# xu-ji/IIC

Hardware: AMD Instinct MI355X
Metric: paired-images/sec, STL10 96x96 ClusterNet5g+IID_loss (higher is better)
Workload: dtype bf16; 1 GPU; STL10 96x96 ClusterNet5g IID+ (cluster_sobel.py train step), batch 660 pairs/GPU, 5 sub-heads, k=70, bf16 MFMA convs / fp32 stem+heads+loss, fused HIP Adam; global_batch_pairs=660, input=96x96x1 grey -> sobel 2ch, parallelism=dp1, streams=2, launch=hip-graph replay: 6 linear graph segments, the two views on two streams

## Files before the change

iic_amd/csrc/conv_igemm_bd.hip:

```cpp
#include "common.h"
#include "conv_plan.h"
#include "conv_tile.h"
#include "../../include/iic_hip.h"

__device__ __forceinline__ void bd_bload(u32x4& d, const unsigned char* p) {
  asm volatile("global_load_dwordx4 %0, %1, off" : "=v"(d) : "v"(p) : "memory");
}
template <int N>
__device__ __forceinline__ void bd_bwait(u32x4& d) {
  asm volatile("s_waitcnt vmcnt(%1)" : "+v"(d) : "i"(N) : "memory");
}


#define BD_BM 256
#define BD_BN 128
#define BD_THREADS 256
#define BD_PROF_SLOTS 16
#ifndef BD_STORE_UB
#define BD_STORE_UB 8
#endif

template <bool GATHER, int ABL, int MS, int RED, int WN = 2, bool PAD = false>
__device__ __forceinline__ void bd_tile(
    const iic_conv_geom& g, const bf16_t* __restrict__ in, const unsigned char* __restrict__ wfrag,
    bf16_t* __restrict__ out, float* __restrict__ stats, const bf16_t* __restrict__ res_grad,
    const bf16_t* __restrict__ res_act, int accumulate, int lds_a_bytes,
    const bf16_t* __restrict__ red_y, const float* __restrict__ red_coef,
    const bf16_t* __restrict__ red_y2, float* __restrict__ red_stats, float* __restrict__ red_stats2,
    unsigned long long* __restrict__ prof, int blk_in_class, int nwg_class, const bd_blk& B) {
  constexpr int BNT = WN * 64, NWM = 4 / WN;
  constexpr bool CANBLK = !GATHER && MS * 32 * (4 / WN) == 256;
  const bool blk = CANBLK && !PAD && B.bw > 0;
  constexpr int CLD = BNT + 8;
  constexpr bool PROF = (ABL & 128) != 0;
  static_assert(!(PAD && GATHER), "the padded patch is a multi-tap form");
  constexpr bool SWZ = !PAD;
  unsigned long long t_stamp[8];
  unsigned long long t_bsum = 0, t_b0 = 0;
  int t_nb = 0;
  if (PROF) t_stamp[0] = __builtin_readcyclecounter();
  constexpr int BM = MS * 32 * NWM, WR = MS * 32;
  extern __shared__ __attribute__((aligned(16))) unsigned char smem_raw[];
  unsigned char* sA = smem_raw;
  int* s_pin = reinterpret_cast<int*>(smem_raw + lds_a_bytes);
  int* s_pout = s_pin + BM;
  float* s_red = reinterpret_cast<float*>(s_pout + BM);
  unsigned char* s_key = reinterpret_cast<unsigned char*>(s_red + NWM * 2 * BNT);
  bf16_t* sC = reinterpret_cast<bf16_t*>(smem_raw);

  const int tid = threadIdx.x, lane = tid & 63;
  const int wave = __builtin_amdgcn_readfirstlane(tid >> 6);
  const int wm = WN == 2 ? wave >> 1 : wave, wn = WN == 2 ? wave & 1 : 0;
  const int l31 = lane & 31, g5 = lane >> 5;

  const int nt = g.Cout / BNT;
  const int tix = xcd_tile_index(blk_in_class, nwg_class);
  const int mtile = tix / nt, ntile = tix - mtile * nt;
  const int n0 = ntile * BNT;
  const int m0 = mtile * BM;
  const int in_pixels = g.N * g.in_Hp * g.in_Wp;

  int v_tapoff = g.tap_off[lane & (IIC_MAX_TAPS - 1)];
  const int v_tapw = g.tap_w[lane & (IIC_MAX_TAPS - 1)];
  int blk_glo = 0;
  bool blk_full = true;
  if (blk) {
    const int tpi = B.nbx * B.nby;
    const int bn = mtile / tpi, brem = mtile - bn * tpi;
    const int by = brem / B.nbx, bx = brem - by * B.nbx;
    const int y0 = by * B.bh, x0 = bx * B.bw;
    blk_glo = (bn * g.in_Hp + y0 + g.oy) * g.in_Wp + x0 + g.ox;
    blk_full = y0 + B.bh <= g.MY && x0 + B.bw <= g.MX && B.bw * B.bh == BM;
    v_tapoff = (v_tapoff / g.in_Wp) * B.PW + v_tapoff % g.in_Wp;
    if (tid < BM) {
      int ky = tid / B.bw;
      const int kx = tid - ky * B.bw;
      const int y = y0 + ky, x = x0 + kx;
      const bool valid = ky < B.bh && y < g.MY && x < g.MX;
      ky = ky < B.bh ? ky : B.bh - 1;
      s_pin[tid] = ky * B.PW + kx;
      s_pout[tid] = valid ? (bn * g.out_Hp + y + g.py) * g.out_Wp + x + g.px : -1;
    }
  } else if (tid < BM) {
    int pin, pout;
    igemm_row_pixels(g, m0 + tid, pin, pout);
    s_pin[tid] = pin;
    s_pout[tid] = pout;
  }
  __syncthreads();
  const int p_lo = blk ? 0 : s_pin[0];
  const int npix = GATHER ? BM : (blk ? B.npix : (BM >= 192 ? g.NP256 : g.NP));
  const int keyw = blk ? B.PW : g.in_Wp;
  const int jskip = blk ? B.PW - B.bw
                        : ((!GATHER && g.sx == 1 && ((g.in_Wp - g.MX) & 1) == 0) ? g.in_Wp - g.MX : 0);
  auto dense_of = [&](int p) { return p - jskip * (p / keyw); };
  int arow[MS];
  int drow[MS];
#pragma unroll
  for (int ms = 0; ms < MS; ++ms) {
    const int row = wm * WR + ms * 32 + l31;
    const int pr = GATHER ? row : (s_pin[row] - p_lo);
    arow[ms] = SWZ ? pr : pr * ROWB + g5 * 16;
    drow[ms] = (SWZ && !GATHER) ? dense_of(s_pin[row]) : pr;
  }
  if (SWZ && !GATHER && jskip != 0) {
    for (int r = tid; r < npix; r += BD_THREADS) s_key[r] = (unsigned char)((dense_of(p_lo + r) >> 1) & 7);
    __syncthreads();
  }
  const int v_tapd = v_tapoff - jskip * (v_tapoff / keyw);
  const int nblk = (npix * 128 + 1023) >> 10;
  const int dma_rl = lane / 9, dma_pc = min(lane - dma_rl * 9, 7) * 8;
  auto dma_patch = [&](int c0) {
    if (PAD) {
      const int nj = (npix + PT144_ROWS - 1) / PT144_ROWS;
      for (int j = wave; j < nj; j += BD_THREADS / 64) {
        long p = (long)p_lo + j * PT144_ROWS + dma_rl;
        p = p < in_pixels ? p : in_pixels - 1;
        __builtin_amdgcn_global_load_lds(
            (const __attribute__((address_space(1))) void*)(in + (p * g.Cin + c0 + dma_pc)),
            (__attribute__((address_space(3))) void*)(sA + j * PT144_PIECE), 16, 0, 0);
      }
      asm volatile("s_waitcnt vmcnt(0)" ::: "memory");
      return;
    }
    for (int kb = wave; kb < nblk; kb += BD_THREADS / 64) {
      const int q = kb * 64 + lane;
      const int r = q >> 3;
      const int ls = (q & 7) ^ (GATHER ? ((r >> 1) & 7)
                                       : (jskip != 0 ? (int)s_key[r < npix ? r : npix - 1]
                                                     : (((p_lo + r) >> 1) & 7)));
      long p = GATHER ? (long)s_pin[r < BM ? r : BM - 1] : (long)p_lo + r;
      if (blk) {
        const int rc = r < npix ? r : npix - 1;
        const int py = (rc * B.mul) >> 16;
        p = (long)blk_glo + py * g.in_Wp + (rc - py * B.PW);
      }
      p = p < in_pixels ? p : in_pixels - 1;
      __builtin_amdgcn_global_load_lds(
          (const __attribute__((address_space(1))) void*)(in + (p * g.Cin + c0 + ls * 8)),
          (__attribute__((address_space(3))) void*)(sA + kb * 1024), 16, 0, 0);
    }
    asm volatile("s_waitcnt vmcnt(0)" ::: "memory");
  };
  auto a_base = [&](int R, int D) { return R * 128 + (((g5 ^ (D >> 1)) & 1) << 4); };
  auto a_kk = [&](int D) { return ((D >> 2) & 3) << 5; };

  f32x16 acc[MS][2];
#pragma unroll
  for (int ms = 0; ms < MS; ++ms)
#pragma unroll
    for (int ns = 0; ns < 2; ++ns)
#pragma unroll
      for (int r = 0; r < 16; ++r) acc[ms][ns][r] = 0.f;

  const int nchunks = g.Cin >> 6;
  const int ntaps = g.ntaps;
  const int NIT = nchunks * ntaps;
  const long frag_it = (long)(g.Cout >> 5) * 4096;
  const unsigned char* wb0 = wfrag + (long)((n0 + wn * 64) >> 5) * 4096 + lane * 16;
  auto frag_ptr = [&](int tap, int chunk) {
    const int tw = __builtin_amdgcn_readlane(v_tapw, tap);
    return wb0 + ((long)tw * nchunks + chunk) * frag_it;
  };

  if (PROF) t_stamp[1] = __builtin_readcyclecounter();
  u32x4 Bc[4][2];
  {
    const unsigned char* p = frag_ptr(0, 0);
#pragma unroll
    for (int ks = 0; ks < 4; ++ks)
#pragma unroll
      for (int ns = 0; ns < 2; ++ns)
        bd_bload(Bc[ks][ns], p + ns * 4096 + ks * 1024);
  }
  dma_patch(0);
  __syncthreads();
  if (PROF) t_stamp[2] = __builtin_readcyclecounter();

  int tap = 0, chunk = 0;
  bf16x8 a[2][MS];
  int pcur[MS], kcur[MS];
#pragma unroll
  for (int ms = 0; ms < MS; ++ms) {
    const int t0 = GATHER ? 0 : __builtin_amdgcn_readlane(v_tapoff, 0);
    if (SWZ) {
      const int R = arow[ms] + t0;
      const int D = drow[ms] + (GATHER ? 0 : __builtin_amdgcn_readlane(v_tapd, 0));
      pcur[ms] = a_base(R, D);
      kcur[ms] = a_kk(D);
      a[0][ms] = *reinterpret_cast<const bf16x8*>(sA + pcur[ms] + kcur[ms]);
    } else {
      pcur[ms] = arow[ms] + t0 * ROWB;
      kcur[ms] = 0;
      a[0][ms] = *reinterpret_cast<const bf16x8*>(sA + pcur[ms]);
    }
  }
  for (int it = 0; it < NIT; ++it) {
    int tn = tap + 1, cn = chunk;
    if (tn == ntaps) { tn = 0; ++cn; }
    const bool more = (it + 1 < NIT);
    if (!more) { tn = tap; cn = chunk; }
    const unsigned char* nb = (ABL & 2) ? frag_ptr(0, 0) : frag_ptr(tn, cn);
    const int toffn = GATHER ? 0 : __builtin_amdgcn_readlane(v_tapoff, tn);
    const int tdn = GATHER ? 0 : __builtin_amdgcn_readlane(v_tapd, tn);
    int pnext[MS], knext[MS];
#pragma unroll
    for (int ms = 0; ms < MS; ++ms) {
      if (SWZ) {
        const int R = arow[ms] + toffn;
        const int D = drow[ms] + tdn;
        pnext[ms] = a_base(R, D);
        knext[ms] = a_kk(D);
      } else {
        pnext[ms] = arow[ms] + toffn * ROWB;
        knext[ms] = 0;
      }
    }
    auto a_read = [&](int ks, int nxt, int cur, int ms) {
      if (!(ABL & 16)) {
        if (SWZ)
          a[nxt][ms] = (ks < 3) ? *reinterpret_cast<const bf16x8*>(sA + pcur[ms] + (((ks + 1) << 5) ^ kcur[ms]))
                                : *reinterpret_cast<const bf16x8*>(sA + pnext[ms] + knext[ms]);
        else
          a[nxt][ms] = (ks < 3) ? *reinterpret_cast<const bf16x8*>(sA + pcur[ms] + (ks + 1) * 32)
                                : *reinterpret_cast<const bf16x8*>(sA + pnext[ms]);
      } else {
        a[nxt][ms] = a[cur][ms];
      }
    };
#pragma unroll
    for (int ks = 0; ks < 4; ++ks) {
      const int cur = ks & 1, nxt = cur ^ 1;
      bd_bwait<7>(Bc[ks][0]);
      __builtin_amdgcn_sched_barrier(0);
      const bf16x8 b0 = __builtin_bit_cast(bf16x8, Bc[ks][0]);
#pragma unroll
      for (int ms = 0; ms < MS; ++ms) {
        acc[ms][0] = __builtin_amdgcn_mfma_f32_32x32x16_bf16(a[cur][ms], b0, acc[ms][0], 0, 0, 0);
        a_read(ks, nxt, cur, ms);
        __builtin_amdgcn_sched_barrier(0);
      }
      bd_bwait<6>(Bc[ks][1]);
      bd_bload(Bc[ks][0], nb + ks * 1024);
      __builtin_amdgcn_sched_barrier(0);
      const bf16x8 b1 = __builtin_bit_cast(bf16x8, Bc[ks][1]);
#pragma unroll
      for (int ms = 0; ms < MS; ++ms)
        acc[ms][1] = __builtin_amdgcn_mfma_f32_32x32x16_bf16(a[cur][ms], b1, acc[ms][1], 0, 0, 0);
      __builtin_amdgcn_sched_barrier(0);
      bd_bload(Bc[ks][1], nb + 4096 + ks * 1024);
      __builtin_amdgcn_sched_barrier(0);
    }
#pragma unroll
    for (int ms = 0; ms < MS; ++ms) {
      pcur[ms] = pnext[ms];
      kcur[ms] = knext[ms];
    }
    if (more && tn == 0 && !(ABL & 8)) {
      if (PROF) t_b0 = __builtin_readcyclecounter();
      __syncthreads();
      if (!(ABL & 1)) dma_patch(cn * 64);
      __syncthreads();
      if (PROF) { t_bsum += __builtin_readcyclecounter() - t_b0; ++t_nb; }
#pragma unroll
      for (int ms = 0; ms < MS; ++ms)
        a[0][ms] = *reinterpret_cast<const bf16x8*>(sA + pcur[ms] + (SWZ ? kcur[ms] : 0));
    }
    tap = tn;
    chunk = cn;
  }

  asm volatile("s_waitcnt vmcnt(0)" ::: "memory");
  if (PROF) t_stamp[3] = __builtin_readcyclecounter();
  if (ABL & 4) {
    float t = 0.f;
#pragma unroll
    for (int ms = 0; ms < MS; ++ms)
#pragma unroll
      for (int ns = 0; ns < 2; ++ns)
#pragma unroll
        for (int r = 0; r < 16; ++r) t += acc[ms][ns][r];
    if (t == 123.f) out[0] = 1;
    return;
  }
  const bool tail = blk ? !blk_full : igemm_tile_has_invalid(g, m0, BM);
  if (stats && !(ABL & 64)) {
    if (tail) {
#pragma unroll
      for (int ms = 0; ms < MS; ++ms)
#pragma unroll
        for (int r = 0; r < 16; ++r)
          if (s_pout[wm * WR + ms * 32 + mfma32_row(r, lane)] < 0) {
            acc[ms][0][r] = 0.f;
            acc[ms][1][r] = 0.f;
          }
    }
#pragma unroll
    for (int ns = 0; ns < 2; ++ns) {
      f32x2 s2 = {0.f, 0.f}, ss2 = {0.f, 0.f};
#pragma unroll
      for (int ms = 0; ms < MS; ++ms)
#pragma unroll
        for (int r = 0; r < 16; r += 2) {
          const f32x2 v = {acc[ms][ns][r], acc[ms][ns][r + 1]};
          s2 += v;
          ss2 += v * v;
        }
      float s = s2[0] + s2[1], ss = ss2[0] + ss2[1];
      s += __shfl_xor(s, 32, 64);
      ss += __shfl_xor(ss, 32, 64);
      if (lane < 32) {
        const int col = wn * 64 + ns * 32 + lane;
        s_red[(wm * 2 + 0) * BNT + col] = s;
        s_red[(wm * 2 + 1) * BNT + col] = ss;
      }
    }
  }
  __syncthreads();
  if (stats && tid < BNT && !(ABL & 64)) {
    const int stripe = blockIdx.x % IIC_STAT_STRIPES;
    float a0 = 0.f, a1 = 0.f;
#pragma unroll
    for (int q = 0; q < NWM; ++q) {
      a0 += s_red[(q * 2 + 0) * BNT + tid];
      a1 += s_red[(q * 2 + 1) * BNT + tid];
    }
    iic_stat_add(stats, stripe, g.Cout, n0 + tid, 0, a0);
    iic_stat_add(stats, stripe, g.Cout, n0 + tid, 1, a1);
  }
#pragma unroll
  for (int ms = 0; ms < MS; ++ms)
#pragma unroll
    for (int ns = 0; ns < 2; ++ns)
#pragma unroll
      for (int r = 0; r < 16; ++r) {
        const int row = wm * WR + ms * 32 + mfma32_row(r, lane);
        const int col = wn * 64 + ns * 32 + l31;
        sC[row * CLD + col] = f32_to_bf16(acc[ms][ns][r]);
      }
  __syncthreads();
  if (PROF) t_stamp[4] = __builtin_readcyclecounter();
  TileRed tr;
  if (RED) tile_red_zero(tr);
  if (!(ABL & 32))
    igemm_store_tile<BNT, BM, BD_THREADS, 8, RED, (BM == 256 ? BD_STORE_UB : 4)>(sC, s_pout, out, res_grad, res_act, accumulate,
                                                                 g.Cout, n0, tid, red_y, red_coef, red_y2, &tr);
  if (RED)
    igemm_red_finish<BNT, BD_THREADS, RED>(tr, reinterpret_cast<float*>(smem_raw), red_stats, red_stats2,
                                             g.Cout, n0, tid);
  if (PROF && prof && tid == 0) {
    unsigned long long* q = prof + (long)blockIdx.x * BD_PROF_SLOTS;
    const unsigned long long t_end = __builtin_readcyclecounter();
    q[0] = t_stamp[0]; q[1] = t_stamp[1]; q[2] = t_stamp[2]; q[3] = t_stamp[3]; q[4] = t_stamp[4];
    q[5] = t_end; q[6] = t_bsum; q[7] = (unsigned long long)t_nb;
    q[8] = iic_hw_stamp();
    q[9] = (unsigned long long)tix;
    q[10] = __builtin_amdgcn_s_memrealtime();
  }
}

template <bool GATHER, int ABL, int MS, int RED, int WN = 2, bool PAD = false>
__global__ __launch_bounds__(BD_THREADS, ((MS == 4 || WN == 1) ? 2 : 3)) void conv_igemm_bd_kernel(
    const iic_conv_geom g, const bf16_t* __restrict__ in, const unsigned char* __restrict__ wfrag,
    bf16_t* __restrict__ out, float* __restrict__ stats, const bf16_t* __restrict__ res_grad,
    const bf16_t* __restrict__ res_act, int accumulate, int num_mtiles, int lds_a_bytes,
    const bf16_t* __restrict__ red_y, const float* __restrict__ red_coef,
    const bf16_t* __restrict__ red_y2, float* __restrict__ red_stats, float* __restrict__ red_stats2,
    unsigned long long* __restrict__ prof, const bd_blk B) {
  bd_tile<GATHER, ABL, MS, RED, WN, PAD>(g, in, wfrag, out, stats, res_grad, res_act, accumulate, lds_a_bytes, red_y,
                                    red_coef, red_y2, red_stats, red_stats2, prof, (int)blockIdx.x,
                                    num_mtiles * (g.Cout / (WN * 64)), B);
}

__global__ void weight_prep_frag_kernel(const float* __restrict__ w, bf16_t* __restrict__ o, int Co,
                                        int Ci, int T, int mode) {
  const int Nn = mode ? Ci : Co, Kk = mode ? Co : Ci;
  const int n32 = Nn >> 5, nchunks = Kk >> 6;
  const long total = (long)T * Co * Ci;
  for (long i = (long)blockIdx.x * blockDim.x + threadIdx.x; i < total;
       i += (long)gridDim.x * blockDim.x) {
    const int e = (int)(i & 7), lane = (int)((i >> 3) & 63), ks = (int)((i >> 9) & 3);
    long r = i >> 11;
    const int j = (int)(r % n32);
    r /= n32;
    const int kc = (int)(r % nchunks), t = (int)(r / nchunks);
    const int n = j * 32 + (lane & 31), k = kc * 64 + ks * 16 + (lane >> 5) * 8 + e;
    const int co = mode ? k : n, ci = mode ? n : k;
    o[i] = f32_to_bf16(w[((long)co * Ci + ci) * T + t]);
  }
}

IIC_SWITCH(g_p64_enabled, 1, iic_debug_enable_p64)
IIC_SWITCH(g_p64_red, 0, iic_debug_p64_red)

extern "C" {

#ifdef IIC_DEBUG_HOOKS
static unsigned long long* g_bd_prof = nullptr;
IIC_HOOK void iic_debug_bd_prof(void* buf) { g_bd_prof = (unsigned long long*)buf; }
IIC_HOOK int iic_debug_bd_prof_slots(void) { return BD_PROF_SLOTS; }
#else
static constexpr unsigned long long* g_bd_prof = nullptr;
#endif

static long bd_lds(long npix, int rows, int couts, bool pad, bool keys, int* lds_a = nullptr) {
  const long a = pad ? pt144_bytes(npix) : (npix * 128 + 1023) & ~1023L;
  const long c = (long)rows * (couts + 8) * 2;
  const long la = ((a > c ? a : c) + 15) & ~15L;
  if (lds_a) *lds_a = (int)la;
  return la + 2L * rows * 4 + 4L * BD_BN * 4 + (keys ? (npix + 15) & ~15L : 0);
}
static long bd_lds_rows(const iic_conv_geom* g, int ms, int wn = 2, bool pad = false, int* lds_a = nullptr) {
  const int rows = ms * 32 * (4 / wn);
  const long npix = g->ntaps == 1 ? rows : (rows >= 192 ? g->NP256 : g->NP);
  const bool skip = g->ntaps > 1 && g->sx == 1 && ((g->in_Wp - g->MX) & 1) == 0 && g->in_Wp != g->MX;
  return bd_lds(npix, rows, wn * 64, pad, !pad && skip, lds_a);
}
IIC_SWITCH(g_bd_pitch144, IIC_BD_PITCH144, iic_debug_bd_pitch144)
#ifdef IIC_DEBUG_HOOKS
IIC_HOOK int iic_debug_get_bd_pitch144(void) { return g_bd_pitch144; }
#endif
static bool bd_pad_ok(const iic_conv_geom* g, int ms) {
  if (!g_bd_pitch144 || g->ntaps < 2 || g->sx != 1 || g->sy != 1) return false;
  return bd_lds_rows(g, ms, 2, true) <= (ms == 4 ? IIC_LDS_WG2 : IIC_LDS_WG3);
}
IIC_SWITCH(g_bd_w1, 1, iic_debug_bd_w1)
static bool bd_w1_ok(const iic_conv_geom* g) {
  return g_bd_w1 && g->Cout % 64 == 0 && g->Cout % BD_BN != 0 && g->ntaps > 1 && g->NP256 > 0 &&
         bd_lds_rows(g, 2, 1) <= IIC_LDS_BYTES;
}
IIC_SWITCH(g_bd_ms, 0, iic_debug_bd_ms)
static int bd_pick_ms(const iic_conv_geom* g) {
  const bool ok4 = (g->ntaps == 1 || g->NP256 > 0) && bd_lds_rows(g, 4) <= IIC_LDS_BYTES;
  const bool ok2 = (g->ntaps == 1 || g->NP > 0) && bd_lds_rows(g, 2) <= IIC_LDS_BYTES;
  if (g_bd_ms == 4) return ok4 ? 4 : (ok2 ? 2 : 0);
  if (g_bd_ms == 2) return ok2 ? 2 : (ok4 ? 4 : 0);
  if (ok4 && ok2 && g->ntaps > 1) {
    const long M = igemm_rows_host(g);
    if (((M + 255) / 256) * (g->Cout / BD_BN) * 2 <= 512) return 2;
  }
  return ok4 ? 4 : (ok2 ? 2 : 0);
}

IIC_SWITCH(g_bd_blk, 1, iic_debug_bd_blk)
static int bd_block_config(const iic_conv_geom* g, bd_blk* B, int wn) {
  B->bw = 0;
  if (!g_bd_blk || g->ntaps < 2 || g->Cout % (wn * 64) != 0 || g->Cin % 64 != 0) return 0;
  if (g->sy != 1 || g->sx != 1 || g->ty != 1 || g->tx != 1 || g->MY < 32 || g->MX < 32 || g->NP256 <= 0) return 0;
  int mix = 0, miy = 0;
  for (int t = 0; t < g->ntaps; ++t) {
    const int iy = g->tap_off[t] / g->in_Wp, ix = g->tap_off[t] % g->in_Wp;
    if (ix > 8 || iy > 8) return 0;
    mix = ix > mix ? ix : mix;
    miy = iy > miy ? iy : miy;
  }
  if (mix & 1) return 0;
  double best = -1.0;
  int best_bw = 0;
  long best_tiles = 0;
  for (int bw = 8; bw <= 64 && bw <= g->MX; ++bw) {
    const int bh = BD_BM / bw;
    if (bh < 2 || bh > g->MY) continue;
    const long tiles = (long)((g->MX + bw - 1) / bw) * ((g->MY + bh - 1) / bh);
    const long npix = (long)(bw + mix) * (bh + miy);
    if (bd_lds(npix, BD_BM, wn * 64, false, true) > IIC_LDS_WG2 || npix >= 65536 / (bw + mix)) continue;
    const double cost = (double)tiles * (1.0 + 0.5 * (double)npix * 128.0 / 32768.0);
    if (best < 0 || cost < best) { best = cost; best_bw = bw; best_tiles = tiles; }
  }
  if (best < 0) return 0;
  const int bw = best_bw, bh = BD_BM / bw;
  if ((double)g->MY * g->MX < 0.88 * (double)BD_BM * (double)best_tiles) return 0;
  const int npix = (bw + mix) * (bh + miy);
  if (g_bd_blk != 2 && !(bd_lds_rows(g, wn == 2 ? 4 : 2, wn) > IIC_LDS_WG2 || npix * 10 < g->NP256 * 7)) return 0;
  B->bw = bw; B->bh = bh;
  B->nbx = (g->MX + bw - 1) / bw; B->nby = (g->MY + bh - 1) / bh;
  B->PW = bw + mix; B->npix = npix; B->mul = (65536 + B->PW - 1) / B->PW;
  return 1;
}

static bool conv_make_plan(const iic_conv_geom* g, conv_plan* p) {
  *p = conv_plan{};
  if (!g) return false;
  if (g_p64_enabled && iic_p64_plan(g, p)) {
    p->red_ok = g_p64_red != 0;
    return true;
  }
  if (g->Cin % 64 != 0 || g->Cout % 64 != 0 || g->ntaps < 1 || g->ntaps > IIC_MAX_TAPS) return false;
  const int abl = iic_debug_get_ablate();
  if (abl == 0 && g_bd_ms == 0 && iic_pw_plan(g, p)) {
    p->red_ok = true;
    return true;
  }
  p->wn = g->Cout % BD_BN != 0 ? 1 : 2;
  const bool blocked = (p->wn == 1 || abl == 0) && bd_block_config(g, &p->blk, p->wn) != 0;
  if (p->wn == 1) p->ms = (blocked || bd_w1_ok(g)) ? 2 : 0;
  else p->ms = blocked ? 4 : bd_pick_ms(g);
  if (p->ms == 0) {
    *p = conv_plan{};
    return false;
  }
  const int rows = p->ms * 32 * (4 / p->wn);
  p->gather = g->ntaps == 1;
  p->red_ok = !p->gather;
  p->pad = p->wn == 2 && !blocked && abl == 0 && bd_pad_ok(g, p->ms);
  p->mtiles = blocked ? g->N * p->blk.nbx * p->blk.nby : (int)((igemm_rows_host(g) + rows - 1) / rows);
  p->grid = p->mtiles * (g->Cout / (p->wn * 64));
  p->lds = blocked ? bd_lds(p->blk.npix, BD_BM, p->wn * 64, false, true, &p->lds_a)
                   : bd_lds_rows(g, p->ms, p->wn, p->pad, &p->lds_a);
  p->kernel = CONV_BD;
  return true;
}

int iic_conv_igemm_frag_supported(const iic_conv_geom* g) {
  conv_plan p;
  return conv_make_plan(g, &p) ? 1 : 0;
}

int iic_conv_igemm_red_supported(const iic_conv_geom* g) {
  conv_plan p;
  return conv_make_plan(g, &p) && p.red_ok ? 1 : 0;
}

int iic_conv_igemm_frag_red(const iic_conv_geom* g, const void* in, const void* wfrag, void* out,
                            float* stats, const void* res_grad, const void* res_act, int accumulate,
                            const void* red_y, const float* red_coef, const void* red_y2,
                            float* red_stats, float* red_stats2, void* stream);

int iic_conv_igemm_frag(const iic_conv_geom* g, const void* in, const void* wfrag, void* out,
                        float* stats, const void* res_grad, const void* res_act, int accumulate,
                        void* stream) {
  return iic_conv_igemm_frag_red(g, in, wfrag, out, stats, res_grad, res_act, accumulate, nullptr, nullptr,
                                 nullptr, nullptr, nullptr, stream);
}

int iic_conv_igemm_frag_red(const iic_conv_geom* g, const void* in, const void* wfrag, void* out,
                            float* stats, const void* res_grad, const void* res_act, int accumulate,
                            const void* red_y, const float* red_coef, const void* red_y2,
                            float* red_stats, float* red_stats2, void* stream) {
  if (!g || !in || !wfrag || !out) return IIC_ERR_ARG;
  if ((red_y == nullptr) != (red_stats == nullptr) || (red_y2 == nullptr) != (red_stats2 == nullptr) ||
      (red_y2 && !red_y) || (red_coef && !red_y))
    return IIC_ERR_ARG;
  const int red = red_y ? (red_y2 ? 2 : 1) : 0;
  if (!(accumulate & IIC_ACC_PREMASK) && (res_grad == nullptr) != (res_act == nullptr)) return IIC_ERR_ARG;
  conv_plan p;
  if (!conv_make_plan(g, &p)) return IIC_ERR_UNSUPPORTED;
  if (p.kernel == CONV_P64) {
    if (red && !p.red_ok) return IIC_ERR_UNSUPPORTED;
    return iic_p64_launch(g, p, in, wfrag, out, stats, res_grad, res_act, accumulate, red_y, red_coef, red_y2,
                          red_stats, red_stats2, stream);
  }
  if (p.kernel == CONV_PW)
    return iic_pw_launch(g, p, in, wfrag, out, stats, res_grad, res_act, accumulate, red_y, red_coef, red_y2, red_stats,
// ... 136 lines not shown
```

iic_amd/csrc/conv_igemm_p64.hip:

```cpp
#include "common.h"
#include "conv_plan.h"
#include "conv_tile.h"
#include "../../include/iic_hip.h"

#define P64_BM 256
#define P64_BN 64
#define P64_THREADS 512
#define P64_NT 9
#define P64_CLD P64_BN
#define P64_SC_BYTES(BM_) ((BM_) * P64_CLD * 2)
#define P64_NTAB 4
#define P64_TAB_BYTES(BM_) (P64_NTAB * (BM_) * (4 + 2))

struct P64Walk {
  int n, y, x;
};
__device__ __forceinline__ void p64_walk_init(P64Walk& w, const iic_conv_geom& g, int m) {
  const int plane = g.MY * g.MX;
  w.n = m / plane;
  const int r = m - w.n * plane;
  w.y = r / g.MX;
  w.x = r - w.y * g.MX;
}
__device__ __forceinline__ void p64_walk_advance(P64Walk& w, const iic_conv_geom& g, int d_y, int d_x) {
  w.x += d_x;
  w.y += d_y;
  if (w.x >= g.MX) { w.x -= g.MX; ++w.y; }
  while (w.y >= g.MY) { w.y -= g.MY; ++w.n; }
}
__device__ __forceinline__ void p64_walk_pixels(const P64Walk& w, const iic_conv_geom& g, int& pin,
                                                int& pout) {
  const bool valid = w.n < g.N;
  const int n = valid ? w.n : g.N - 1, y = valid ? w.y : g.MY - 1, x = valid ? w.x : g.MX - 1;
  pin = (n * g.in_Hp + y * g.sy + g.oy) * g.in_Wp + x * g.sx + g.ox;
  pout = valid ? (n * g.out_Hp + y * g.ty + g.py) * g.out_Wp + x * g.tx + g.px : -1;
}

template <int ABL, int RED>
__global__ __launch_bounds__(512) void conv_igemm_p64_kernel(
    const iic_conv_geom g, const bf16_t* __restrict__ in, const unsigned char* __restrict__ wfrag,
    bf16_t* __restrict__ out, float* __restrict__ stats, const bf16_t* __restrict__ res_grad,
    const bf16_t* __restrict__ res_act, int accumulate, int num_tiles, int pb_bytes, int max_tap_off,
    const bf16_t* __restrict__ red_y, const float* __restrict__ red_coef,
    const bf16_t* __restrict__ red_y2, float* __restrict__ red_stats, float* __restrict__ red_stats2,
    unsigned long long* __restrict__ prof) {
  constexpr bool PROF = (ABL & 8) != 0;
  constexpr int NW = 8, BM = P64_BM;
  constexpr int NWM = BM / 64;
  constexpr int SC_BYTES = BM * P64_CLD * 2, TAB_ROWS = P64_NTAB * BM;
  unsigned long long ph[6] = {0, 0, 0, 0, 0, 0}, t_a = 0, t_b = 0, t_loop = 0;
  extern __shared__ __attribute__((aligned(16))) unsigned char smem_raw[];
  unsigned char* const sP0 = smem_raw;
  unsigned char* const sP1 = smem_raw + pb_bytes;
  bf16_t* const sC = reinterpret_cast<bf16_t*>(smem_raw + 2 * pb_bytes);
  int* const s_pout = reinterpret_cast<int*>(smem_raw + 2 * pb_bytes + SC_BYTES);
  unsigned short* const s_prow = reinterpret_cast<unsigned short*>(s_pout + TAB_ROWS);
  float* const s_red = reinterpret_cast<float*>(sC);

  constexpr int NTH = NW * 64;
  constexpr int NCO = 1;
  const int tid = threadIdx.x, lane = tid & 63;
  const int wave = __builtin_amdgcn_readfirstlane(tid >> 6);
  const int wm = wave >> 1, wn = wave & 1;
  const int l31 = lane & 31, g5 = lane >> 5;
  const int M = g.N * g.MY * g.MX;
  const int in_pixels = g.N * g.in_Hp * g.in_Wp;

  const int G = gridDim.x;
  const int wl = xcd_tile_index(blockIdx.x, G);
  const int t0 = (int)(((long)wl * num_tiles) / G), t1 = (int)(((long)(wl + 1) * num_tiles) / G);
  if (t0 >= t1) return;

  const int v_tapoff = g.tap_off[lane & (IIC_MAX_TAPS - 1)];
  const int d_y = BM / g.MX, d_x = BM - d_y * g.MX;

  P64Walk wr, w0, w255;
  p64_walk_init(wr, g, t0 * BM + (tid & (BM - 1)));
  p64_walk_init(w0, g, t0 * BM);
  p64_walk_init(w255, g, t0 * BM + BM - 1);
  int plo_q[3], nblk_q[3];
  auto tabulate = [&](int t) {
    int pin, pout, p0, p255, dummy;
    p64_walk_pixels(w0, g, p0, dummy);
    p64_walk_pixels(w255, g, p255, dummy);
    p0 = __builtin_amdgcn_readfirstlane(p0);
    p255 = __builtin_amdgcn_readfirstlane(p255);
    if (tid < BM) {
      p64_walk_pixels(wr, g, pin, pout);
      s_pout[(t & (P64_NTAB - 1)) * BM + tid] = pout;
      s_prow[(t & (P64_NTAB - 1)) * BM + tid] = (unsigned short)(pin - p0);
    }
    p64_walk_advance(wr, g, d_y, d_x);
    p64_walk_advance(w0, g, d_y, d_x);
    p64_walk_advance(w255, g, d_y, d_x);
    plo_q[0] = plo_q[1];
    nblk_q[0] = nblk_q[1];
    plo_q[1] = plo_q[2];
    nblk_q[1] = nblk_q[2];
    plo_q[2] = p0;
    nblk_q[2] = ((p255 + max_tap_off - p0 + 1) * 128 + 1023) >> 10;
  };
  auto dma_issue = [&](unsigned char* dst, int plo, int nblk) {
    for (int blk = wave; blk < nblk; blk += NW) {
      const int q = blk * 64 + lane;
      const int r = q >> 3;
      const int ls = (q & 7) ^ ((r >> 1) & 7);
      int p = plo + r;
      p = p < in_pixels ? p : in_pixels - 1;
      __builtin_amdgcn_global_load_lds(
          (const __attribute__((address_space(1))) void*)(in + ((long)p * 64 + ls * 8)),
          (__attribute__((address_space(3))) void*)(dst + blk * 1024), 16, 0, 0);
    }
  };

  tabulate(t0);
  tabulate(t0 + 1);
  dma_issue(sP0, plo_q[1], nblk_q[1]);
  u32x4 Bw[P64_NT][NCO][4];
#pragma unroll
  for (int tap = 0; tap < P64_NT; ++tap)
#pragma unroll
    for (int c = 0; c < NCO; ++c) {
      const unsigned char* p = wfrag + ((long)g.tap_w[tap] * 2 + wn + c) * 4096 + lane * 16;
#pragma unroll
      for (int ks = 0; ks < 4; ++ks) Bw[tap][c][ks] = *reinterpret_cast<const u32x4*>(p + ks * 1024);
    }
  f32x2 st_s[NCO], st_ss[NCO];
#pragma unroll
  for (int c = 0; c < NCO; ++c) {
    st_s[c] = f32x2{0.f, 0.f};
    st_ss[c] = f32x2{0.f, 0.f};
  }
  TileRed tr;
  if (RED) tile_red_zero(tr);

  if (PROF) t_loop = __builtin_readcyclecounter();
  for (int t = t0; t < t1; ++t) {
    const int par = (t - t0) & 1;
    unsigned char* const sP = par ? sP1 : sP0;
    if (PROF) t_a = __builtin_readcyclecounter();
    asm volatile("s_waitcnt vmcnt(0)" ::: "memory");
    __syncthreads();
    if (PROF) { t_b = __builtin_readcyclecounter(); ph[0] += t_b - t_a; t_a = t_b; }
    const bool spread = RED == 0 && !res_grad && !res_act && !accumulate;
    if (t > t0 && !(ABL & 2) && !spread)
      igemm_store_tile<P64_BN, BM, NTH, 0, RED, (RED ? 1 : 4)>(sC, s_pout + ((t - 1) & (P64_NTAB - 1)) * BM,
                                                            out, res_grad, res_act, accumulate, P64_BN, 0, tid,
                                                            red_y, red_coef, red_y2, &tr);
    if (PROF) { t_b = __builtin_readcyclecounter(); ph[1] += t_b - t_a; t_a = t_b; }
    if (t + 1 < t1 && !(ABL & 1)) dma_issue(par ? sP0 : sP1, plo_q[2], nblk_q[2]);
    tabulate(t + 2);
    if (PROF) { t_b = __builtin_readcyclecounter(); ph[2] += t_b - t_a; t_a = t_b; }
    int R0[2];
#pragma unroll
    for (int ms = 0; ms < 2; ++ms)
      R0[ms] = s_prow[(t & (P64_NTAB - 1)) * BM + wm * 64 + ms * 32 + l31];
    f32x16 acc[2][NCO];
    constexpr int NTAPS = (ABL & 4) ? 1 : P64_NT;
    auto load_a = [&](int tap, bf16x8 (&a)[2][4]) {
      const int toff = __builtin_amdgcn_readlane(v_tapoff, tap);
#pragma unroll
      for (int ms = 0; ms < 2; ++ms) {
        const int R = R0[ms] + toff;
        const int key = (R >> 1) & 7;
        const int base = R * 128 + (((g5 ^ key) & 1) << 4);
        const int kk = (key >> 1) << 5;
#pragma unroll
        for (int ks = 0; ks < 4; ++ks)
          a[ms][ks] = *reinterpret_cast<const bf16x8*>(sP + base + ((ks << 5) ^ kk));
      }
    };
#pragma unroll
    for (int tap = 0; tap < NTAPS; ++tap) {
      bf16x8 a[2][4];
      load_a(tap, a);
      if (spread && t > t0 && !(ABL & 2)) {
        constexpr int SIT = BM * 8 / NTH;
        constexpr int PER = (SIT + P64_NT - 2) / (P64_NT - 1);
#pragma unroll
        for (int q = 0; q < PER; ++q) {
          const int it = (tap - 1) * PER + q;
          if (tap >= 1 && it < SIT) {
            const int idx = tid + it * NTH;
            const int row = idx >> 3, ch = idx & 7;
            const int po = s_pout[((t - 1) & (P64_NTAB - 1)) * BM + row];
            if (po >= 0)
              *reinterpret_cast<uint4*>(out + (long)po * P64_BN + ch * 8) =
                  *reinterpret_cast<const uint4*>(sC + row * P64_CLD + ch * 8);
          }
        }
      }
#pragma unroll
      for (int ks = 0; ks < 4; ++ks)
#pragma unroll
        for (int c = 0; c < NCO; ++c) {
          const bf16x8 b = __builtin_bit_cast(bf16x8, Bw[tap][c][ks]);
          if (tap == 0 && ks == 0) {
            const f32x16 z = {0.f, 0.f, 0.f, 0.f, 0.f, 0.f, 0.f, 0.f, 0.f, 0.f, 0.f, 0.f, 0.f, 0.f, 0.f, 0.f};
            acc[0][c] = __builtin_amdgcn_mfma_f32_32x32x16_bf16(a[0][ks], b, z, 0, 0, 0);
            acc[1][c] = __builtin_amdgcn_mfma_f32_32x32x16_bf16(a[1][ks], b, z, 0, 0, 0);
          } else {
            acc[0][c] = __builtin_amdgcn_mfma_f32_32x32x16_bf16(a[0][ks], b, acc[0][c], 0, 0, 0);
            acc[1][c] = __builtin_amdgcn_mfma_f32_32x32x16_bf16(a[1][ks], b, acc[1][c], 0, 0, 0);
          }
        }
    }
    if (stats) {
      if ((t + 1) * BM > M) {
#pragma unroll
        for (int ms = 0; ms < 2; ++ms)
#pragma unroll
          for (int r = 0; r < 16; ++r)
            if (t * BM + wm * 64 + ms * 32 + mfma32_row(r, lane) >= M) {
#pragma unroll
              for (int c = 0; c < NCO; ++c) acc[ms][c][r] = 0.f;
            }
      }
#pragma unroll
      for (int c = 0; c < NCO; ++c)
#pragma unroll
        for (int ms = 0; ms < 2; ++ms)
#pragma unroll
          for (int r = 0; r < 16; r += 2) {
            const f32x2 v = {acc[ms][c][r], acc[ms][c][r + 1]};
            st_s[c] += v;
            st_ss[c] += v * v;
          }
    }
    if (PROF) { t_b = __builtin_readcyclecounter(); ph[3] += t_b - t_a; t_a = t_b; }
    asm volatile("s_waitcnt lgkmcnt(0)" ::: "memory");
    __builtin_amdgcn_s_barrier();
    if (PROF) { t_b = __builtin_readcyclecounter(); ph[4] += t_b - t_a; t_a = t_b; }
#pragma unroll
    for (int c = 0; c < NCO; ++c)
#pragma unroll
      for (int ms = 0; ms < 2; ++ms)
#pragma unroll
        for (int r = 0; r < 16; ++r)
          sC[(wm * 64 + ms * 32 + mfma32_row(r, lane)) * P64_CLD + (wn + c) * 32 + l31] = f32_to_bf16(acc[ms][c][r]);
    if (PROF) { t_b = __builtin_readcyclecounter(); ph[5] += t_b - t_a; }
  }
  if (PROF && prof && tid == 0) {
    unsigned long long* q = prof + (long)blockIdx.x * 8;
#pragma unroll
    for (int i = 0; i < 6; ++i) q[i] = ph[i];
    q[6] = (unsigned long long)(t1 - t0);
    q[7] = __builtin_readcyclecounter() - t_loop;
  }

  __syncthreads();
  if (!(ABL & 2))
    igemm_store_tile<P64_BN, BM, NTH, 0, RED, (RED ? 1 : 4)>(sC, s_pout + ((t1 - 1) & (P64_NTAB - 1)) * BM, out,
                                                          res_grad, res_act, accumulate, P64_BN, 0, tid,
                                                          red_y, red_coef, red_y2, &tr);
  if (RED)
    igemm_red_finish<P64_BN, NTH, RED>(tr, reinterpret_cast<float*>(sC), red_stats, red_stats2, P64_BN,
                                               0, tid);
  if (stats) {
    __syncthreads();
#pragma unroll
    for (int c = 0; c < NCO; ++c) {
      float s1 = st_s[c][0] + st_s[c][1], s2 = st_ss[c][0] + st_ss[c][1];
      s1 += __shfl_xor(s1, 32, 64);
      s2 += __shfl_xor(s2, 32, 64);
      if (lane < 32) {
        s_red[(wm * 2 + 0) * P64_BN + (wn + c) * 32 + lane] = s1;
        s_red[(wm * 2 + 1) * P64_BN + (wn + c) * 32 + lane] = s2;
      }
    }
    __syncthreads();
    if (tid < P64_BN) {
      float a0 = 0.f, a1 = 0.f;
#pragma unroll
      for (int q = 0; q < NWM; ++q) {
        a0 += s_red[(q * 2 + 0) * P64_BN + tid];
        a1 += s_red[(q * 2 + 1) * P64_BN + tid];
      }
      const int stripe = blockIdx.x % IIC_STAT_STRIPES;
      iic_stat_add(stats, stripe, P64_BN, tid, 0, a0);
      iic_stat_add(stats, stripe, P64_BN, tid, 1, a1);
    }
  }
}

#ifdef IIC_DEBUG_HOOKS
static unsigned long long* g_p64_prof = nullptr;
IIC_HOOK void iic_debug_p64_prof(void* buf) { g_p64_prof = (unsigned long long*)buf; }
#else
static constexpr unsigned long long* g_p64_prof = nullptr;
#endif
IIC_SWITCH(g_p64_grid, 0, iic_debug_p64_grid)

static long p64_pb_bytes(const iic_conv_geom* g, int bm = P64_BM) {
  return (((long)(bm == 128 ? g->NP : g->NP256) * 128) + 1023) & ~1023L;
}

bool iic_p64_plan(const iic_conv_geom* g, conv_plan* p) {
  if (g->Cin != 64 || g->Cout != 64 || g->ntaps != P64_NT || g->NP256 <= 0 || g->NP256 > 65535) return false;
  if (!igemm_dense_host(g)) return false;
  const long lds = 2 * p64_pb_bytes(g) + P64_SC_BYTES(P64_BM) + P64_TAB_BYTES(P64_BM);
  if (lds > IIC_LDS_BYTES) return false;
  const long nt = ((long)g->N * g->MY * g->MX + P64_BM - 1) / P64_BM;
  const int ncu = g_p64_grid > 0 ? g_p64_grid : iic_num_cus();
  p->kernel = CONV_P64;
  p->mtiles = (int)nt;
  p->grid = nt < ncu ? (int)nt : ncu;
  p->lds_a = (int)p64_pb_bytes(g);
  p->lds = lds;
  return true;
}

int iic_p64_launch(const iic_conv_geom* g, const conv_plan& p, const void* in, const void* wfrag, void* out, float* stats,
                   const void* res_grad, const void* res_act, int accumulate, const void* red_y,
                   const float* red_coef, const void* red_y2, float* red_stats, float* red_stats2,
                   void* stream) {
  const int red = red_y ? (red_y2 ? 2 : 1) : 0;
  const long M = (long)g->N * g->MY * g->MX;
  if (M <= 0) return IIC_ERR_ARG;
  if (M >= (1L << 31) - P64_BM || (long)g->N * g->in_Hp * g->in_Wp >= (1L << 31)) return IIC_ERR_UNSUPPORTED;
  int mto = 0;
  for (int i = 0; i < g->ntaps; ++i) mto = g->tap_off[i] > mto ? g->tap_off[i] : mto;
  int rc = IIC_OK;
#define P64_LAUNCH2(AB_, RD_)                                                                          \
  rc = iic_launch_lds<conv_igemm_p64_kernel<AB_, RD_>>(                                                \
      dim3(p.grid), dim3(512), p.lds, (hipStream_t)stream, *g, (const bf16_t*)in,                      \
      (const unsigned char*)wfrag, (bf16_t*)out, stats, (const bf16_t*)res_grad,                       \
      (const bf16_t*)res_act, accumulate, p.mtiles, p.lds_a, mto, (const bf16_t*)red_y, red_coef,      \
      (const bf16_t*)red_y2, red_stats, red_stats2, g_p64_prof)
#define P64_LAUNCH(AB_) P64_LAUNCH2(AB_, 0)
  if (red == 1) P64_LAUNCH2(0, 1);
  else if (red == 2) P64_LAUNCH2(0, 2);
  else {
    switch (iic_debug_get_ablate()) {
#ifdef IIC_BD_ABLATIONS
      case 1: P64_LAUNCH(1); break;
      case 2: P64_LAUNCH(2); break;
      case 3: P64_LAUNCH(3); break;
      case 4: P64_LAUNCH(4); break;
      case 7: P64_LAUNCH(7); break;
      case 8: P64_LAUNCH(8); break;
#endif
      default: P64_LAUNCH(0); break;
    }
  }
  return rc ? rc : iic_launch_status();
}
```

Baseline: 19130 paired-images/sec.

## Use SGPR-base addressing for weight loads and interleave p64 DMA/tabulation into tap loop

In the bd kernel, weight fragment loads now use a scalar base plus a per-lane vector offset and an immediate offset, which removes per-load 64-bit address arithmetic in VGPRs. In the p64 kernel, a new FORM path computes row indices incrementally, issues global-to-LDS DMA through a scalar-base helper, and moves the next tile's DMA issue and tabulation inside the tap loop so they overlap with MFMA work. A-fragment LDS addresses are now built with precomputed swizzle bit tricks. This adds inline asm that saves and restores m0 and a more complex schedule, and R0 is now prefetched at the end of each tile.

```diff
diff --git a/iic_amd/csrc/conv_igemm_bd.hip b/iic_amd/csrc/conv_igemm_bd.hip
--- a/iic_amd/csrc/conv_igemm_bd.hip
+++ b/iic_amd/csrc/conv_igemm_bd.hip
@@ -3,8 +3,17 @@
 #include "conv_tile.h"
 #include "../../include/iic_hip.h"
 
-__device__ __forceinline__ void bd_bload(u32x4& d, const unsigned char* p) {
-  asm volatile("global_load_dwordx4 %0, %1, off" : "=v"(d) : "v"(p) : "memory");
+template <int OFF>
+__device__ __forceinline__ void bd_bload_at(u32x4& d, unsigned voff, const unsigned char* sbase) {
+  asm volatile("global_load_dwordx4 %0, %1, %2 offset:%3" : "=v"(d) : "v"(voff), "s"(sbase), "n"(OFF) : "memory");
+}
+__device__ __forceinline__ void bd_bload(u32x4& d, unsigned voff, const unsigned char* sbase, int ks) {
+  switch (ks) {
+    case 0: bd_bload_at<0>(d, voff, sbase); break;
+    case 1: bd_bload_at<1024>(d, voff, sbase); break;
+    case 2: bd_bload_at<2048>(d, voff, sbase); break;
+    default: bd_bload_at<3072>(d, voff, sbase); break;
+  }
 }
 template <int N>
 __device__ __forceinline__ void bd_bwait(u32x4& d) {
@@ -157,7 +166,8 @@
   const int ntaps = g.ntaps;
   const int NIT = nchunks * ntaps;
   const long frag_it = (long)(g.Cout >> 5) * 4096;
-  const unsigned char* wb0 = wfrag + (long)((n0 + wn * 64) >> 5) * 4096 + lane * 16;
+  const unsigned char* wb0 = wfrag + (long)((n0 + wn * 64) >> 5) * 4096;
+  const unsigned bvoff = (unsigned)lane * 16u;
   auto frag_ptr = [&](int tap, int chunk) {
     const int tw = __builtin_amdgcn_readlane(v_tapw, tap);
     return wb0 + ((long)tw * nchunks + chunk) * frag_it;
@@ -171,7 +181,7 @@
     for (int ks = 0; ks < 4; ++ks)
 #pragma unroll
       for (int ns = 0; ns < 2; ++ns)
-        bd_bload(Bc[ks][ns], p + ns * 4096 + ks * 1024);
+        bd_bload(Bc[ks][ns], bvoff, p + ns * 4096, ks);
   }
   dma_patch(0);
   __syncthreads();
@@ -241,14 +251,14 @@
         __builtin_amdgcn_sched_barrier(0);
       }
       bd_bwait<6>(Bc[ks][1]);
-      bd_bload(Bc[ks][0], nb + ks * 1024);
+      bd_bload(Bc[ks][0], bvoff, nb, ks);
       __builtin_amdgcn_sched_barrier(0);
       const bf16x8 b1 = __builtin_bit_cast(bf16x8, Bc[ks][1]);
 #pragma unroll
       for (int ms = 0; ms < MS; ++ms)
         acc[ms][1] = __builtin_amdgcn_mfma_f32_32x32x16_bf16(a[cur][ms], b1, acc[ms][1], 0, 0, 0);
       __builtin_amdgcn_sched_barrier(0);
-      bd_bload(Bc[ks][1], nb + 4096 + ks * 1024);
+      bd_bload(Bc[ks][1], bvoff, nb + 4096, ks);
       __builtin_amdgcn_sched_barrier(0);
     }
 #pragma unroll
diff --git a/iic_amd/csrc/conv_igemm_p64.hip b/iic_amd/csrc/conv_igemm_p64.hip
--- a/iic_amd/csrc/conv_igemm_p64.hip
+++ b/iic_amd/csrc/conv_igemm_p64.hip
@@ -36,7 +36,37 @@
   pout = valid ? (n * g.out_Hp + y * g.ty + g.py) * g.out_Wp + x * g.tx + g.px : -1;
 }
 
-template <int ABL, int RED>
+struct P64Row {
+  int n, y, x, pin, pout;
+};
+struct P64Step {
+  int d_n, d_y, d_x, MY, MX, pin_step, pin_xw, pin_yw, pout_step, pout_xw, pout_yw;
+};
+__device__ __forceinline__ void p64_row_init(P64Row& r, const iic_conv_geom& g, int m) {
+  P64Walk w;
+  p64_walk_init(w, g, m);
+  r.n = w.n; r.y = w.y; r.x = w.x;
+  r.pin = (w.n * g.in_Hp + w.y * g.sy + g.oy) * g.in_Wp + w.x * g.sx + g.ox;
+  r.pout = (w.n * g.out_Hp + w.y * g.ty + g.py) * g.out_Wp + w.x * g.tx + g.px;
+}
+__device__ __forceinline__ void p64_row_advance(P64Row& r, const P64Step& s) {
+  r.n += s.d_n; r.y += s.d_y; r.x += s.d_x; r.pin += s.pin_step; r.pout += s.pout_step;
+  const bool cx = r.x >= s.MX;
+  r.x -= cx ? s.MX : 0; r.y += cx ? 1 : 0; r.pin += cx ? s.pin_xw : 0; r.pout += cx ? s.pout_xw : 0;
+  const bool cy = r.y >= s.MY;
+  r.y -= cy ? s.MY : 0; r.n += cy ? 1 : 0; r.pin += cy ? s.pin_yw : 0; r.pout += cy ? s.pout_yw : 0;
+}
+
+__device__ __forceinline__ void p64_dma16s(unsigned voff, const unsigned char* sbase, unsigned lds_dst) {
+  unsigned keep;
+  asm volatile(
+      "s_mov_b32 %0, m0\n\ts_mov_b32 m0, %3\n\ts_nop 0\n\tglobal_load_lds_dwordx4 %1, %2\n\ts_mov_b32 m0, %0"
+      : "=&s"(keep)
+      : "v"(voff), "s"(sbase), "s"(lds_dst)
+      : "memory");
+}
+
+template <int ABL, int RED, bool FORM>
 __global__ __launch_bounds__(512) void conv_igemm_p64_kernel(
     const iic_conv_geom g, const bf16_t* __restrict__ in, const unsigned char* __restrict__ wfrag,
     bf16_t* __restrict__ out, float* __restrict__ stats, const bf16_t* __restrict__ res_grad,
@@ -45,6 +75,7 @@
     const bf16_t* __restrict__ red_y2, float* __restrict__ red_stats, float* __restrict__ red_stats2,
     unsigned long long* __restrict__ prof) {
   constexpr bool PROF = (ABL & 8) != 0;
+  constexpr bool BK = FORM && RED == 0;
   constexpr int NW = 8, BM = P64_BM;
   constexpr int NWM = BM / 64;
   constexpr int SC_BYTES = BM * P64_CLD * 2, TAB_ROWS = P64_NTAB * BM;
@@ -63,6 +94,10 @@
   const int wave = __builtin_amdgcn_readfirstlane(tid >> 6);
   const int wm = wave >> 1, wn = wave & 1;
   const int l31 = lane & 31, g5 = lane >> 5;
+  const uint32_t g5x = (uint32_t)g5 << 4;
+  typedef const bf16x8 __attribute__((address_space(3))) * lds_frag_ptr;
+  const uint32_t lds_base = __builtin_amdgcn_readfirstlane(
+      (uint32_t)(uintptr_t)(__attribute__((address_space(3))) unsigned char*)smem_raw);
   const int M = g.N * g.MY * g.MX;
   const int in_pixels = g.N * g.in_Hp * g.in_Wp;
 
@@ -113,9 +148,77 @@
     }
   };
 
-  tabulate(t0);
-  tabulate(t0 + 1);
-  dma_issue(sP0, plo_q[1], nblk_q[1]);
+  P64Step stp;
+  P64Row rr, r0, r255;
+  int pin_last = 0;
+  uint32_t lane_src = 0;
+  if (BK) {
+    const int plane = g.MY * g.MX;
+    stp.d_n = BM / plane;
+    const int rem = BM - stp.d_n * plane;
+    stp.d_y = rem / g.MX;
+    stp.d_x = rem - stp.d_y * g.MX;
+    stp.MY = g.MY; stp.MX = g.MX;
+    stp.pin_step = (stp.d_n * g.in_Hp + stp.d_y * g.sy) * g.in_Wp + stp.d_x * g.sx;
+    stp.pin_xw = g.sy * g.in_Wp - g.MX * g.sx;
+    stp.pin_yw = (g.in_Hp - g.MY * g.sy) * g.in_Wp;
+    stp.pout_step = (stp.d_n * g.out_Hp + stp.d_y * g.ty) * g.out_Wp + stp.d_x * g.tx;
+    stp.pout_xw = g.ty * g.out_Wp - g.MX * g.tx;
+    stp.pout_yw = (g.out_Hp - g.MY * g.ty) * g.out_Wp;
+    pin_last = ((g.N - 1) * g.in_Hp + (g.MY - 1) * g.sy + g.oy) * g.in_Wp + (g.MX - 1) * g.sx + g.ox;
+    p64_row_init(rr, g, t0 * BM + (tid & (BM - 1)));
+    p64_row_init(r0, g, t0 * BM);
+    p64_row_init(r255, g, t0 * BM + BM - 1);
+    lane_src = (uint32_t)(lane >> 3) * 128u + (uint32_t)(((lane & 7) ^ (lane >> 4) ^ ((wave & 1) << 2)) << 4);
+  }
+  auto tabulate1 = [&](int t) {
+    const int p0 = r0.n < g.N ? r0.pin : pin_last;
+    const int p255 = r255.n < g.N ? r255.pin : pin_last;
+    if (wave < BM / 64) {
+      const bool valid = rr.n < g.N;
+      s_pout[(t & (P64_NTAB - 1)) * BM + tid] = valid ? rr.pout : -1;
+      s_prow[(t & (P64_NTAB - 1)) * BM + tid] = (unsigned short)((valid ? rr.pin : pin_last) - p0);
+      p64_row_advance(rr, stp);
+    }
+    p64_row_advance(r0, stp);
+    p64_row_advance(r255, stp);
+    plo_q[0] = plo_q[1];
+    nblk_q[0] = nblk_q[1];
+    plo_q[1] = plo_q[2];
+    nblk_q[1] = nblk_q[2];
+    plo_q[2] = p0;
+    nblk_q[2] = ((p255 + max_tap_off - p0 + 1) * 128 + 1023) >> 10;
+  };
+  auto dma_issue1 = [&](uint32_t dst, int plo, int nblk) {
+    const unsigned char* const ing = reinterpret_cast<const unsigned char*>(in);
+    for (int blk = wave; blk < nblk; blk += NW) {
+      const int rb = plo + blk * 8;
+      const unsigned char* src = ing + (long)rb * 128;
+      uint32_t vo = lane_src;
+      if (rb + 7 >= in_pixels) {
+        const int rc = rb < in_pixels ? rb : in_pixels - 1;
+        int p = rb + (lane >> 3);
+        p = p < in_pixels ? p : in_pixels - 1;
+        src = ing + (long)rc * 128;
+        vo = (uint32_t)(p - rc) * 128u + (lane_src & 127u);
+      }
+      p64_dma16s(vo, src, dst + (uint32_t)blk * 1024u);
+    }
+  };
+  int R0[2];
+
+  if (BK) {
+    tabulate1(t0);
+    tabulate1(t0 + 1);
+    __syncthreads();
+#pragma unroll
+    for (int ms = 0; ms < 2; ++ms) R0[ms] = s_prow[(t0 & (P64_NTAB - 1)) * BM + wm * 64 + ms * 32 + l31];
+    dma_issue1(lds_base, plo_q[1], nblk_q[1]);
+  } else {
+    tabulate(t0);
+    tabulate(t0 + 1);
+    dma_issue(sP0, plo_q[1], nblk_q[1]);
+  }
   u32x4 Bw[P64_NT][NCO][4];
 #pragma unroll
   for (int tap = 0; tap < P64_NT; ++tap)
@@ -148,17 +251,37 @@
                                                             out, res_grad, res_act, accumulate, P64_BN, 0, tid,
                                                             red_y, red_coef, red_y2, &tr);
     if (PROF) { t_b = __builtin_readcyclecounter(); ph[1] += t_b - t_a; t_a = t_b; }
-    if (t + 1 < t1 && !(ABL & 1)) dma_issue(par ? sP0 : sP1, plo_q[2], nblk_q[2]);
-    tabulate(t + 2);
+    if (!BK) {
+      if (t + 1 < t1 && !(ABL & 1)) dma_issue(par ? sP0 : sP1, plo_q[2], nblk_q[2]);
+      tabulate(t + 2);
+    }
     if (PROF) { t_b = __builtin_readcyclecounter(); ph[2] += t_b - t_a; t_a = t_b; }
-    int R0[2];
-#pragma unroll
-    for (int ms = 0; ms < 2; ++ms)
-      R0[ms] = s_prow[(t & (P64_NTAB - 1)) * BM + wm * 64 + ms * 32 + l31];
+    if (!BK) {
+#pragma unroll
+      for (int ms = 0; ms < 2; ++ms)
+        R0[ms] = s_prow[(t & (P64_NTAB - 1)) * BM + wm * 64 + ms * 32 + l31];
+    }
+    const uint32_t pbase = lds_base + (par ? (uint32_t)pb_bytes : 0u);
+    const int prow = (int)(pbase >> 7);
+    const uint32_t kfix = (pbase >> 4) & 0x40u;
     f32x16 acc[2][NCO];
     constexpr int NTAPS = (ABL & 4) ? 1 : P64_NT;
     auto load_a = [&](int tap, bf16x8 (&a)[2][4]) {
       const int toff = __builtin_amdgcn_readlane(v_tapoff, tap);
+      if (FORM) {
+        const int toffp = toff + prow;
+#pragma unroll
+        for (int ms = 0; ms < 2; ++ms) {
+          uint32_t tt = (uint32_t)(R0[ms] + toffp) << 3;
+          asm volatile("" : "+v"(tt));
+          uint32_t u = (tt << 4) | (tt & 0x70u);
+          asm volatile("" : "+v"(u));
+#pragma unroll
+          for (int ks = 0; ks < 4; ++ks)
+            a[ms][ks] = *reinterpret_cast<const lds_frag_ptr>((uintptr_t)(u ^ g5x ^ ((uint32_t)(ks << 5) ^ kfix)));
+        }
+        return;
+      }
 #pragma unroll
       for (int ms = 0; ms < 2; ++ms) {
         const int R = R0[ms] + toff;
@@ -174,6 +297,10 @@
     for (int tap = 0; tap < NTAPS; ++tap) {
       bf16x8 a[2][4];
       load_a(tap, a);
+      if (BK) {
+        if (tap == 0 && t + 1 < t1 && !(ABL & 1)) dma_issue1(lds_base + (par ? 0u : (uint32_t)pb_bytes), plo_q[2], nblk_q[2]);
+        if (tap == (NTAPS > 6 ? 6 : NTAPS - 1)) tabulate1(t + 2);
+      }
       if (spread && t > t0 && !(ABL & 2)) {
         constexpr int SIT = BM * 8 / NTH;
         constexpr int PER = (SIT + P64_NT - 2) / (P64_NT - 1);
@@ -238,6 +365,10 @@
 #pragma unroll
         for (int r = 0; r < 16; ++r)
           sC[(wm * 64 + ms * 32 + mfma32_row(r, lane)) * P64_CLD + (wn + c) * 32 + l31] = f32_to_bf16(acc[ms][c][r]);
+    if (BK && t + 1 < t1) {
+#pragma unroll
+      for (int ms = 0; ms < 2; ++ms) R0[ms] = s_prow[((t + 1) & (P64_NTAB - 1)) * BM + wm * 64 + ms * 32 + l31];
+    }
     if (PROF) { t_b = __builtin_readcyclecounter(); ph[5] += t_b - t_a; }
   }
   if (PROF && prof && tid == 0) {
@@ -290,6 +421,7 @@
 static constexpr unsigned long long* g_p64_prof = nullptr;
 #endif
 IIC_SWITCH(g_p64_grid, 0, iic_debug_p64_grid)
+IIC_SWITCH(g_p64_form, 1, iic_debug_p64_form)
 
 static long p64_pb_bytes(const iic_conv_geom* g, int bm = P64_BM) {
   return (((long)(bm == 128 ? g->NP : g->NP256) * 128) + 1023) & ~1023L;
@@ -321,12 +453,21 @@
   int mto = 0;
   for (int i = 0; i < g->ntaps; ++i) mto = g->tap_off[i] > mto ? g->tap_off[i] : mto;
   int rc = IIC_OK;
-#define P64_LAUNCH2(AB_, RD_)                                                                          \
-  rc = iic_launch_lds<conv_igemm_p64_kernel<AB_, RD_>>(                                                \
+#define P64_LAUNCH3(AB_, RD_, FM_)                                                                     \
+  rc = iic_launch_lds<conv_igemm_p64_kernel<AB_, RD_, FM_>>(                                           \
       dim3(p.grid), dim3(512), p.lds, (hipStream_t)stream, *g, (const bf16_t*)in,                      \
       (const unsigned char*)wfrag, (bf16_t*)out, stats, (const bf16_t*)res_grad,                       \
       (const bf16_t*)res_act, accumulate, p.mtiles, p.lds_a, mto, (const bf16_t*)red_y, red_coef,      \
       (const bf16_t*)red_y2, red_stats, red_stats2, g_p64_prof)
+#ifdef IIC_DEBUG_HOOKS
+#define P64_LAUNCH2(AB_, RD_)                                                                          \
+  do {                                                                                                 \
+    if (g_p64_form) P64_LAUNCH3(AB_, RD_, true);                                                       \
+    else P64_LAUNCH3(AB_, RD_, false);                                                                 \
+  } while (0)
+#else
+#define P64_LAUNCH2(AB_, RD_) P64_LAUNCH3(AB_, RD_, true)
+#endif
 #define P64_LAUNCH(AB_) P64_LAUNCH2(AB_, 0)
   if (red == 1) P64_LAUNCH2(0, 1);
   else if (red == 2) P64_LAUNCH2(0, 2);
```

After: 19520 paired-images/sec, median of 6. 1.02x the previous value.
